# sair-lab/AirSLAM

Hardware: AMD Instinct MI355X
Metric: stereo detect+match pairs/sec (2x PLNet @512x512 internal: points + lines, junctions on the left + LightGlue match) (higher is better)
Workload: dtype fp16

## Files before the change

### airslam_amd/_lib.py

```python
from __future__ import annotations

import ctypes as C
import os

_HERE = os.path.dirname(os.path.abspath(__file__))
LIB_PATH = os.path.join(_HERE, "libairfe.so")


class Tuning(C.Structure):
    _fields_ = [(n, C.c_int) for n in (
        "fuse_lg_block", "gemm_small_max_m", "gemm8_min_m", "gemmr_min_m", "gemmr_wgs", "qkv_pair", "block_min_m", "lgb_tokens", "sg_kenc_gemm",
        "fold_qkv", "overlap_lines", "kf_graph", "kf_spec_rows", "fuse_dec", "assign_fused", "fold_out_proj", "desc_gather_stream", "copy_wgs")] + [("reserved", C.c_int * 5)]


class Cfg(C.Structure):
    _fields_ = [
        ("device", C.c_int), ("precision", C.c_int), ("max_batch", C.c_int), ("enc_chunk", C.c_int),
        ("max_keypoints", C.c_int), ("keypoint_threshold", C.c_float), ("remove_borders", C.c_int),
        ("nms_radius", C.c_int), ("line_threshold", C.c_float), ("line_length_threshold", C.c_float),
        ("matcher", C.c_int), ("image_width", C.c_int), ("image_height", C.c_int), ("sinkhorn_iters", C.c_int),
        ("superpoint_pack", C.c_char_p), ("plnet_s1_pack", C.c_char_p), ("lightglue_pack", C.c_char_p),
        ("superglue_pack", C.c_char_p), ("matcher_precision", C.c_int), ("line_precision", C.c_int), ("check_launches", C.c_int),
        ("tuning", C.POINTER(Tuning)),
    ]


class Stage0(C.Structure):
# ... 188 lines not shown
    "airfe_stereo_points": (C.c_int, [C.c_void_p, C.c_void_p, C.c_void_p, C.c_int, C.c_void_p, C.c_int, C.c_void_p, C.c_int, C.c_void_p, C.c_void_p,
                                      C.c_void_p, C.POINTER(C.c_int)]),
    "airfe_stereo_points_batch_dev": (C.c_int, [C.c_void_p] * 6 + [C.c_int, C.c_int, C.c_void_p, C.c_void_p, C.c_int] + [C.c_void_p] * 5),
    "airfe_track_pose_batch_dev": (C.c_int, [C.c_void_p, C.c_void_p, C.c_void_p, C.c_int, C.c_void_p, C.c_int, C.c_void_p, C.c_void_p, C.c_int, C.c_int,
                                             C.c_void_p, C.c_void_p, C.c_void_p, C.c_void_p, C.c_void_p]),
    "airfe_frame_optimize": (C.c_int, [C.c_void_p, C.c_void_p, C.c_void_p, C.c_int] + [C.c_void_p] * 7 + [C.POINTER(C.c_int)]),
    "airfe_frame_optimize_batch_dev": (C.c_int, [C.c_void_p, C.c_void_p, C.c_void_p, C.c_void_p, C.c_int, C.c_int] + [C.c_void_p] * 9),
    "airfe_track_pose_opt_batch_dev": (C.c_int, [C.c_void_p, C.c_void_p, C.c_void_p, C.c_int, C.c_void_p, C.c_int, C.c_void_p, C.c_int, C.c_void_p,
                                                 C.c_void_p, C.c_int, C.c_int] + [C.c_void_p] * 9),
    "airfe_sync": (C.c_int, [C.c_void_p]),
    "airfe_superglue_status": (C.c_int, [C.c_void_p, C.c_void_p]),
    "airfe_profile_enable": (C.c_int, [C.c_void_p, C.c_int]),
    "airfe_profile_stages": (C.c_int, []),
    "airfe_profile_stage_name": (C.c_char_p, [C.c_int]),
    "airfe_profile_read": (C.c_int, [C.c_void_p, C.c_void_p, C.c_void_p, C.c_void_p, C.c_void_p]),
    "airfe_debug_detector_maps": (C.c_int, [C.c_void_p, C.c_int, C.c_void_p, C.c_void_p, C.c_void_p]),
    "airfe_debug_lightglue_scores": (C.c_int, [C.c_void_p, C.c_void_p, C.c_int, C.c_void_p, C.c_int, C.c_void_p]),
    "airfe_debug_superglue_scores": (C.c_int, [C.c_void_p, C.c_void_p, C.c_int, C.c_void_p, C.c_int, C.c_void_p]),
    "airfe_debug_lg_filter": (C.c_int, [C.c_void_p, C.c_void_p, C.c_int, C.c_int, C.c_void_p, C.c_void_p, C.c_int, C.POINTER(C.c_int)]),
    "airfe_debug_sg_decode": (C.c_int, [C.c_void_p, C.c_void_p, C.c_int, C.c_int, C.c_void_p, C.c_void_p, C.c_void_p, C.c_void_p]),
    "airfe_debug_sg_sinkhorn": (C.c_int, [C.c_void_p, C.c_void_p, C.c_void_p, C.c_int, C.c_int, C.c_float, C.c_int, C.c_int, C.c_void_p, C.POINTER(C.c_int)]),
    "airfe_debug_lg_prepare": (C.c_int, [C.c_void_p, C.POINTER(DebugLgPrepareArgs)]),
    "airfe_debug_lg_assign": (C.c_int, [C.c_void_p, C.POINTER(DebugLgAssignArgs)]),
    "airfe_debug_plnet_stage0": (C.c_int, [C.c_void_p] + [C.c_void_p] * 10),
    "airfe_debug_plnet_s1": (C.c_int, [C.c_void_p, C.POINTER(Stage0), C.c_void_p, C.c_void_p, C.c_int, C.POINTER(C.c_int)]),
    "airfe_debug_plnet_s1_last": (C.c_int, [C.c_void_p, C.c_void_p, C.c_void_p, C.c_int, C.POINTER(C.c_int)]),
    "airfe_debug_preprocess": (C.c_int, [C.c_void_p, C.c_void_p, C.c_int, C.c_int, C.c_int, C.c_void_p]),
    "airfe_debug_conv3x3": (C.c_int, [C.c_void_p, C.c_void_p, C.c_int, C.c_int, C.c_int, C.c_int, C.c_void_p, C.c_void_p,
                                      C.c_int, C.c_int, C.c_void_p]),
    "airfe_debug_conv": (C.c_int, [C.c_void_p, C.POINTER(DebugConvArgs)]),
# ... 38 lines not shown
```

### airslam_amd/api.py

```python
from __future__ import annotations

import ctypes as C
import os
import tempfile
from typing import Dict, Optional

import numpy as np

from . import _lib, weights as W

FEAT = 259


def _pack_arg(x, tmpfiles) -> Optional[bytes]:
    if x is None:
        return None
    if isinstance(x, (str, bytes, os.PathLike)):
        return os.fsencode(x)
    f = tempfile.NamedTemporaryFile(suffix=".airfe", delete=False)
    f.close()
    W.save_pack(f.name, x)
    tmpfiles.append(f.name)
    return f.name.encode()

# ... 387 lines not shown
                                   thr=float(thr), form=int(form), **{k: v.ctypes.data for k, v in out.items()})
        if pad is not None:
            pad = f32(pad)
            a.pad = pad.ctypes.data
        self._chk(self._l.airfe_debug_lg_assign(self._h, C.byref(a)), "airfe_debug_lg_assign")
        return out

    def detector_maps(self, b: int = 1):
        heat = np.empty((b, 512, 512), np.float32)
        nms = np.empty((b, 512, 512), np.float32)
        desc = np.empty((b, 64, 64, 256), np.float32)
        self._chk(self._l.airfe_debug_detector_maps(self._h, b, heat.ctypes.data, nms.ctypes.data, desc.ctypes.data),
                  "airfe_debug_detector_maps")
        return heat, nms, desc

    def debug_preprocess(self, gray):
        gray = np.ascontiguousarray(gray, np.uint8)
        out = np.empty((512, 512), np.float32)
        self._chk(self._l.airfe_debug_preprocess(self._h, gray.ctypes.data, gray.shape[0], gray.shape[1], gray.strides[0],
                                                 out.ctypes.data), "airfe_debug_preprocess")
        return out

    def debug_conv3x3(self, x, w, b, pool=False):
        x = np.ascontiguousarray(x, np.float32); w = np.ascontiguousarray(w, np.float32); b = np.ascontiguousarray(b, np.float32)
        bb, cin, hh, ww = x.shape
        cout = w.shape[0]
        ho, wo = (hh // 2, ww // 2) if pool else (hh, ww)
        y = np.empty((bb, cout, ho, wo), np.float32)
        self._chk(self._l.airfe_debug_conv3x3(self._h, x.ctypes.data, bb, cin, hh, ww, w.ctypes.data, b.ctypes.data, cout,
                                              int(pool), y.ctypes.data), "airfe_debug_conv3x3")
# ... 667 lines not shown
```

### airslam_amd/csrc/airfe.hip

```cpp
#include "airfe_host.h"

namespace airfe_host {
thread_local std::string g_err;

int fail(airfe_ctx* c, const std::string& m) {
  if (c) c->err = m;
  g_err = m;
  return 1;
}

int fail_noexcept(airfe_ctx* c, const char* what, const char* detail) noexcept {
  try {
    std::string m = std::string("airfe: C++ exception at the C boundary (") + what + "): " + (detail ? detail : "unknown");
    if (c) c->err = m;
    g_err = m;
  } catch (...) {
  }
  return 1;
}

int launch_status(airfe_ctx* c) {
  std::string m;
  if (c->launch_err.empty()) {
    const hipError_t e = hipGetLastError();
// ... 158 lines not shown
    if (t->qkv_pair >= 0) c->qkv_pair = t->qkv_pair != 0;
    if (t->block_min_m >= 0) c->block_min = t->block_min_m;
    if (t->lgb_tokens >= 0) {
      if (t->lgb_tokens != 32 && t->lgb_tokens != 64 && t->lgb_tokens != 112 && t->lgb_tokens != 128) { return fail(nullptr, "airfe_create: tuning.lgb_tokens must be 32, 64, 112 or 128"); }
      c->lgb_tokens = t->lgb_tokens;
    }
    if (t->sg_kenc_gemm >= 0) c->sg_kenc_gemm = t->sg_kenc_gemm != 0;
    if (t->fold_qkv >= 0) c->fold_qkv = t->fold_qkv != 0;
    if (t->overlap_lines >= 0) c->overlap_lines = t->overlap_lines != 0;
    if (t->kf_graph >= 0) c->kf_graph_on = t->kf_graph != 0;
    if (t->kf_spec_rows >= 0) c->kf_spec_lines = c->kf_spec_juncs = std::max(t->kf_spec_rows, 1);
    if (t->fuse_dec >= 0) c->fuse_dec = t->fuse_dec != 0;
    if (t->assign_fused >= 0) c->assign_fused = t->assign_fused != 0 ? 1 : 0;
    if (t->fold_out_proj >= 0) c->fold_out = t->fold_out_proj != 0;
    if (t->desc_gather_stream >= 0) c->desc_gather_stream = t->desc_gather_stream != 0;
    if (t->copy_wgs > 0) c->copy_wgs = t->copy_wgs;
  }
  if (hipStreamCreateWithFlags(&c->stream, hipStreamNonBlocking) != hipSuccess ||
      hipStreamCreateWithFlags(&c->stream2, hipStreamNonBlocking) != hipSuccess ||
      hipEventCreateWithFlags(&c->ev_fork, hipEventDisableTiming) != hipSuccess ||
      hipEventCreateWithFlags(&c->ev_join, hipEventDisableTiming) != hipSuccess ||
      hipEventCreateWithFlags(&c->ev_feat, hipEventDisableTiming) != hipSuccess)
    return fail(nullptr, "airfe_create: stream creation failed");
  c->Dmax = (c->prec != 2 && cfg->superpoint_pack && cfg->lightglue_pack) ? 2 * c->Bmax : c->Bmax;
  c->chunk = std::min(std::max(cfg->enc_chunk, 1), c->Dmax);
  c->Lmax = c->Dmax;
  int rc = 0;
  if (cfg->superpoint_pack) rc = load_superpoint(c, cfg->superpoint_pack);
  if (!rc && cfg->lightglue_pack) rc = load_lightglue(c, cfg->lightglue_pack);
  if (!rc && cfg->superglue_pack) rc = load_superglue(c, cfg->superglue_pack);
// ... 585 lines not shown
  }
  if (nlines) *nlines = nl;
  if (njunc) *njunc = nj;
  return 0;
} AIRFE_CATCH(c)

static int plnet_lines_batch(airfe_ctx* c, int B, int h, int w, double* d_lines, int capL, int* d_nlines, float* d_junc, int capJ,
                             int* d_njunc, int nj, int* d_found, hipStream_t st, int phase = 3) {
  if (!c->has_s0 || !c->has_s1) return fail(c, "the batched PLNet path needs the line branch (line.* in the detector pack) and cfg.plnet_s1_pack");
  if (c->prec == 2) return fail(c, "plnet_lines_batch is the 2-byte batch path (fp32 mode goes image by image: plnet_batch_f32)");
  if (B > c->Lmax) return fail(c, "batch exceeds the line-path arena");
  if (capL < 1 || !d_lines || !d_nlines) return fail(c, "detect_plnet_batch: no line output");
  if (nj < 0 || nj > B || (nj > 0 && (!d_junc || !d_njunc || capJ < 1))) return fail(c, "detect_plnet_batch: bad junction arguments");
  if ((phase & 1) && line_branch_dev(c, st, 0, B, false)) return 1;
  bool partial = false;
  if ((phase & 2) && nj > 0 && !c->desc_dense_valid) {
    dense_desc_head(c, nj, st);
    c->desc_dense_valid = true;
    partial = nj != c->last_B;
  }
  int* lfound = d_found ? d_found : c->d_nlines + c->Lmax;
  int* jfound = d_found ? d_found + B : c->d_njunc + c->Lmax;
  const int rc = line_tail_dev(c, 0, B, nullptr, h, w, d_lines, capL, d_nlines, lfound, d_junc, capJ, d_njunc, jfound, nj, st, phase);
  if (partial) c->desc_dense_valid = false;
  return rc;
}

static int plnet_batch_f32(airfe_ctx* c, const uint8_t* d_gray, int B, int h, int w, int stride, size_t img_stride, float* d_feat, int cap, int* d_n,
                           double* d_lines, int capL, int* d_nlines, float* d_junc, int capJ, int* d_njunc, int nj, int* lfound, int* jfound, hipStream_t st) {
  if (!c->has_s0 || !c->has_s1) return fail(c, "the batched PLNet path needs the line branch (line.* in the detector pack) and cfg.plnet_s1_pack");
  if (capL < 1 || !d_lines || !d_nlines) return fail(c, "detect_plnet_batch: no line output");
  if (nj < 0 || nj > B || (nj > 0 && (!d_junc || !d_njunc || capJ < 1))) return fail(c, "detect_plnet_batch: bad junction arguments");
  for (int b = 0; b < B; ++b) {
    const bool jn = b < nj;
    const int rc = detect_dev(c, d_gray + (size_t)b * img_stride, 1, h, w, stride, img_stride, d_feat + (size_t)b * cap * AIRFE_FEAT_DIM, cap, d_n + b, st);
    if (rc || line_branch_dev(c, st, 0, 1, false)) return 1;
    if (line_tail_dev(c, 0, 1, nullptr, h, w, d_lines + (size_t)b * capL * 4, capL, d_nlines + b, lfound ? lfound + b : c->d_nlines + c->Lmax,
                      jn ? d_junc + (size_t)b * capJ * AIRFE_FEAT_DIM : nullptr, capJ, jn ? d_njunc + b : nullptr, jn ? (jfound ? jfound + b : c->d_njunc + c->Lmax) : nullptr,
// ... 570 lines not shown
```

### airslam_amd/csrc/airfe_debug.hip

```cpp
#include "airfe_host.h"

struct DbgTmp {
  airfe_ctx h;
  DbgTmp() {}
  explicit DbgTmp(int prec) { h.prec = h.pack_prec = prec; }
  ~DbgTmp() { for (void* p : h.allocs) (void)hipFree(p); }
};

static std::vector<uint16_t> dbg_conv_x(const float* x, int B, int cin, int H, int W, int prec) {
  std::vector<uint16_t> xin((size_t)B * (H + 2) * (W + 2) * cin, 0);
  for (int bb = 0; bb < B; ++bb)
    for (int ci = 0; ci < cin; ++ci)
      for (int yy = 0; yy < H; ++yy)
        for (int xx = 0; xx < W; ++xx)
          xin[(((size_t)bb * (H + 2) + yy + 1) * (W + 2) + xx + 1) * cin + ci] = cvt2(x[(((size_t)bb * cin + ci) * H + yy) * W + xx], prec);
  return xin;
}
static std::vector<uint16_t> dbg_conv_slabs(const float* w, int cin, int cout, int prec) {
  const int nci = cin / 64;
  return pack_slabs(cout / 64, 9 * nci, prec, [&](int feat, int s, int k) {
    const int tap = s / nci, cc = s % nci, ci = cc * 64 + k;
    return w[((size_t)feat * cin + ci) * 9 + tap];
  });
}
// ... 618 lines not shown
  HIPCHK(c, hipMemcpy2D(a->rowlse, nb, c->rowlse, npb, nb, B, hipMemcpyDeviceToHost));
  HIPCHK(c, hipMemcpy2D(a->collse, nb, c->collse, npb, nb, B, hipMemcpyDeviceToHost));
  HIPCHK(c, hipMemcpy2D(a->rowval, nb, c->rowval, npb, nb, B, hipMemcpyDeviceToHost));
  HIPCHK(c, hipMemcpy2D(a->rowarg, nb, c->rowarg, npb, nb, B, hipMemcpyDeviceToHost));
  HIPCHK(c, hipMemcpy2D(a->colarg, nb, c->colarg, npb, nb, B, hipMemcpyDeviceToHost));
  HIPCHK(c, hipMemcpy(a->idx, didx, (size_t)B * cap * 8, hipMemcpyDeviceToHost));
  HIPCHK(c, hipMemcpy(a->score, dscore, (size_t)B * cap * 4, hipMemcpyDeviceToHost));
  HIPCHK(c, hipMemcpy(a->nmatch, dnm, (size_t)B * 4, hipMemcpyDeviceToHost));
  HIPCHK(c, hipMemsetAsync(c->mdb, 0, M * 256 * 2, st));
  HIPCHK(c, hipMemsetAsync(c->x32, 0, M * 256 * 4, st));
  HIPCHK(c, hipMemsetAsync(c->zbuf, 0, M * 4, st));
  HIPCHK(c, hipStreamSynchronize(st));
  return 0;
} AIRFE_CATCH(c)

}
```

### airslam_amd/csrc/airfe_detect.hip

```cpp
#include "airfe_host.h"

namespace airfe_host {

int ensure_tables(airfe_ctx* c, int h, int w) {
  if (c->tab_w == w && c->tab_h == h) return 0;
  const auto xt = resize_table(AIRFE_INTERNAL_SIZE, w), yt = resize_table(AIRFE_INTERNAL_SIZE, h);
  if (c->tab_w != -1) HIPCHK(c, hipDeviceSynchronize());
  HIPCHK(c, hipMemcpyAsync(c->xtab, xt.data(), xt.size() * 4, hipMemcpyHostToDevice, c->stream));
  HIPCHK(c, hipMemcpyAsync(c->ytab, yt.data(), yt.size() * 4, hipMemcpyHostToDevice, c->stream));
  HIPCHK(c, hipStreamSynchronize(c->stream));
  c->tab_w = w;
  c->tab_h = h;
  return 0;
}

int run_conv(airfe_ctx* c, const ConvW& w, const uint16_t* x, uint16_t* y, int B, int H, int W, int pool, int out_pad,
             hipStream_t st) {
  ConvArgs a;
  a.X = x; a.Wp = w.w; a.bias = w.b; a.Y = y;
  a.B = B; a.H = H; a.W = W; a.CIN = w.cin; a.COUT = w.cout;
  a.pool = pool; a.out_pad = out_pad; a.relu = 1;
  const double px = (double)B * H * W;
  const double ob = px / (pool ? 4 : 1) * w.cout * 2;
  {
// ... 40 lines not shown
}

int dense_desc_head(airfe_ctx* c, int B, hipStream_t st) {
  const int R = AIRFE_INTERNAL_SIZE, cells = B * (R / 8) * (R / 8);
  GemmArgs g;
  g.X1 = c->aDa; g.ld1 = 256; g.K1 = 256; g.Wp = c->cDb.w; g.bias = c->cDb.b;
  g.M = cells; g.N = 256; g.cb_total = c->cDb.cbt; g.epi = EPI_STORE_F32; g.out = c->desc; g.ldo = 256;
  g.small_max = c->gemm_small_max; g.g8_min = c->gemm8_min; g.gr_min = c->gemmr_min; g.gr_wgs = c->gemmr_wgs;
  {
    ProfScope ps(c, ST_HEAD_GEMM, st, 2.0 * cells * 256 * 256, (double)cells * (512 + 1024));
    if (c->desc_gather_stream && cells >= c->gemmr_min && gemmr_gather_applicable(256, g)) launch_gemmr_gather(c->prec, g, st);
    else launch_gemm(c->prec, 256, false, g, st);
  }
  c->desc_normalised = false;
  return c->cfg.check_launches ? launch_status(c) : 0;
}

int detect_dev2(airfe_ctx* c, const uint8_t* d_gray, const uint8_t* d_gray1, int Bs, int h, int w, int stride, size_t img_stride,
                float* d_feat, float* d_feat1, int cap, int* d_n, int* d_n1, hipStream_t st) {
  if (!c->has_sp) return fail(c, "detector weights were not loaded (cfg.superpoint_pack)");
  const int B = d_gray1 ? 2 * Bs : Bs;
  if (Bs < 1 || Bs > c->Bmax || B > c->Dmax) return fail(c, "batch exceeds cfg.max_batch");
  if (h < 1 || w < 1) return fail(c, "empty image");
  if (cap < c->cfg.max_keypoints) return fail(c, "feature capacity < max_keypoints");
  if (ensure_tables(c, h, w)) return 1;
  const int R = AIRFE_INTERNAL_SIZE;
  bool sparse_desc = false;
  if (c->prec == 2) {
    if (d_gray1) return fail(c, "detect_dev2: the fp32 path takes one source");
    if (encode_f32(c, d_gray, B, h, w, stride, img_stride, st)) return 1;
// ... 138 lines not shown
    launch_s0_decode(c->l_head, 160, 128, d + SG_LP, c->l_jloc, nullptr, c->l_joff, d + SG_THIN, d + SG_AUX, chw ? c->s0_loi : nullptr, c->l_ta8, nb,
                     SG_STRIDE, st);
  else
    launch_s0_decode(c->l_dec, 32, 0, d + SG_LP, c->l_jloc, nullptr, c->l_joff, d + SG_THIN, d + SG_AUX, nullptr, c->l_ta8, nb, SG_STRIDE, st);
  const int ccap = F * F;
  hipStream_t s3 = st;
  launch_candidates_nms3(c->l_jloc, nb, F, F, 1e-30f, c->l_cand, c->l_cand_cnt, ccap, s3);
  launch_select_list(c->l_cand, c->l_cand_cnt, ccap, nb, F, 300, 320, c->l_sel, c->l_nsel, s3);
  launch_s0_juncs(c->l_sel, c->l_nsel, c->l_joff, d + SG_JUNCS, 300, 320, nb, SG_STRIDE, s3);
  c->wf_counted = launch_s0_j2l(d + SG_LP, d + SG_JUNCS, 300, NP, 10.0f, d + SG_KEEP, d + SG_MIN, d + SG_MAX, c->wf_counts, nb, SG_STRIDE, chw ? 1 : 0, s3);
  }
  return launch_status(c);
}

int line_tail_dev(airfe_ctx* c, int i0, int nb, const float* loi_chw, int h, int w, double* d_lines, int capL, int* d_nlines, int* d_lfound,
                  float* d_junc, int capJ, int* d_njunc, int* d_jfound, int nj, hipStream_t st, int phase) {
  if (!c->has_s1) return fail(c, "PLNet stage-1 weights were not loaded (cfg.plnet_s1_pack)");
  if (nb < 1 || nb > c->Lmax || nj < 0 || nj > nb) return fail(c, "line path: image range outside the arena");
  const int R = AIRFE_INTERNAL_SIZE, NP = KEEP_CAP;
  float* d = c->s0_stage;
  const float ws = (float)w / (float)R, hs = (float)h / (float)R;
  if (phase & 1) {
  hipStream_t s4 = st;
  if (nj > 0) launch_zero16(c->jmap, (size_t)nj * R * R, s4);
  {
  ProfScope ps(c, ST_PL_STAGE1, st, 0, (double)nb * 49152 * 12);
  launch_wireframe(d + SG_KEEP, d + SG_MIN, d + SG_MAX, NP, 300, c->wf_table, c->wf_keep, c->wf_pairs, c->wf_rep, KEEP_CAP, LINE_CAP,
                   c->wf_counts, c->wf_counted, d + SG_JUNCS, d + SG_LP, c->s1_la, c->wf_prop, nb, SG_STRIDE, s4);
  c->wf_counted = false;
  if (loi_chw) {
    launch_plnet_s1(d + SG_JUNCS, d + SG_LP, c->wf_keep, c->wf_pairs, c->wf_rep, c->wf_counts, loi_chw, 0, nullptr, nullptr, d + SG_THIN, d + SG_AUX,
// ... 15 lines not shown
    } else {
      launch_s1_junc_proj(d + SG_JUNCS, c->l_head, (size_t)128 * 128 * 160, 160, nullptr, 300, c->s1_w[0], c->s1_jfeat, nb, SG_STRIDE, st);
    }
    if (c->cfg.line_precision == 3)
      launch_plnet_s1h(c->wf_pairs, c->wf_counts, c->s1_jfeat, c->l_ta8, c->s1_wsplit, c->s1_w, c->s1_la, c->wf_prop, c->s1_sc, LINE_CAP, nb, st);
    else
      launch_plnet_s1(d + SG_JUNCS, d + SG_LP, c->wf_keep, c->wf_pairs, c->wf_rep, c->wf_counts, nullptr, 0, c->s1_jfeat, c->l_ta8, d + SG_THIN,
                      d + SG_AUX, c->s1_w, c->s1_la, c->s1_sc, KEEP_CAP, LINE_CAP, nb, SG_STRIDE, st);
  }
  }
  ProfScope ps(c, ST_PL_FILTER, st, 0, (double)nb * R * R);
  launch_line_filter(c->s1_la, c->s1_sc, c->wf_counts, c->cfg.remove_borders, c->cfg.line_threshold, c->cfg.line_length_threshold, ws, hs, R,
                     c->jmap, nj, d_lines, capL, d_nlines, d_lfound, LINE_CAP, nb, st);
  }
  if ((phase & 2) && nj > 0) {
    ProfScope ps(c, ST_PL_FILTER, st, 0, (double)nj * R * R * 2);
    const bool from_mask = c->cfg.nms_radius > 0 && !c->nms_map_valid;
    if (from_mask && c->cfg.nms_radius != 4) return fail(c, "line path: the NMS'd score maps of this batch were not kept");
    const float* hsel = (c->cfg.nms_radius > 0 && !from_mask ? c->heat_nms : c->heat) + (size_t)i0 * R * R;
    const unsigned long long* mask = from_mask ? reinterpret_cast<const unsigned long long*>(c->nms_mask) + (size_t)i0 * (R / 8) * (R / 8) : nullptr;
    launch_junction_scan(c->jmap, hsel, R, c->cfg.remove_borders, d_junc, capJ, d_njunc, d_jfound, c->d_njunc + 2 * c->Lmax, nj, st, mask);
    if (!c->desc_dense_valid) return fail(c, "line path: the dense descriptor map of this batch was not made");
    launch_sample_desc(c->desc + (size_t)i0 * (R / 8) * (R / 8) * 256, nj, R / 8, R / 8, d_junc, d_njunc, capJ, ws, hs,
                       c->desc_normalised ? 0 : 1, st);
  }
  return launch_status(c);
}

}
```

### airslam_amd/csrc/airfe_host.h

```cpp
#pragma once
#include "../../include/airfe.h"
#include "../../include/airfe_debug.h"

#include <hip/hip_runtime.h>

#include <algorithm>
#include <cmath>
#include <cstdio>
#include <cstdlib>
#include <cstring>
#include <functional>
#include <map>
#include <string>
#include <vector>

#include "kernels.h"
#include "common.h"

using namespace airfe;


namespace airfe_host {

extern thread_local std::string g_err;
// ... 99 lines not shown
  bool outlier_rejection = false;
  bool nms_map_valid = true;
  int Lmax = 1;
  bool desc_normalised = false;
  int gemm_small_max = 4096, gemm8_min = 16000, gemmr_min = 8192, gemmr_wgs = 256;
  int block_min = 0;
  bool qkv_pair = true;
  int fuse_lg_block = -1;
  int sg_kenc_gemm = -1;
  bool desc_dense_valid = true;
  int last_B = 0;
  int* desc_idx = nullptr;
  int n_cu = 0;
  bool fold_qkv = true;
  bool desc_gather_stream = true;
  bool fold_out = true;

  float *c1a_w = nullptr, *c1a_b = nullptr;
  ConvW c1b, c2a, c2b, c3a, c3b, c4a, c4b, cPa, cDa;
  LinW cPb, cDb;
  float* img32 = nullptr;
  uint16_t *a1b = nullptr, *a2a = nullptr, *a2b = nullptr, *a3a = nullptr, *a3b = nullptr, *a4a = nullptr,
           *a4b = nullptr, *aPa = nullptr, *aDa = nullptr;
  float *logits = nullptr, *heat = nullptr, *heat_nms = nullptr, *nms_tmp = nullptr, *desc = nullptr;
  unsigned char* nms_mask = nullptr;
  int *xtab = nullptr, *ytab = nullptr;
  float* lut = nullptr;
  unsigned long long* cand = nullptr;
  int* cand_cnt = nullptr;
  int tab_w = -1, tab_h = -1;
// ... 180 lines not shown
  uint32_t u = (uint32_t)v << 16;
  float f;
  memcpy(&f, &u, 4);
  return f;
}
bool make_linear(airfe_ctx* c, const float* W, const float* bias, int K, int N, LinW& out, float scale = 1.f,
                 const std::function<int(int)>* src_row = nullptr, const std::function<int(int)>* src_col = nullptr);
int ensure_tables(airfe_ctx* c, int h, int w);
int run_conv(airfe_ctx* c, const ConvW& w, const uint16_t* x, uint16_t* y, int B, int H, int W, int pool, int out_pad, hipStream_t st);
int dense_desc_head(airfe_ctx* c, int B, hipStream_t st);
int detect_dev2(airfe_ctx* c, const uint8_t* d_gray, const uint8_t* d_gray1, int Bs, int h, int w, int stride, size_t img_stride,
                float* d_feat, float* d_feat1, int cap, int* d_n, int* d_n1, hipStream_t st);
int detect_dev(airfe_ctx* c, const uint8_t* d_gray, int B, int h, int w, int stride, size_t img_stride, float* d_feat, int cap, int* d_n, hipStream_t st);
int line_branch_dev(airfe_ctx* c, hipStream_t st, int i0, int nb, bool chw);
int line_tail_dev(airfe_ctx* c, int i0, int nb, const float* loi_chw, int h, int w, double* d_lines, int capL, int* d_nlines, int* d_lfound,
                  float* d_junc, int capJ, int* d_njunc, int* d_jfound, int nj, hipStream_t st, int phase = 3);
void trace(airfe_ctx* c, hipStream_t st, const char* what, size_t li, const char* blk, const void* p, size_t words, unsigned unit_words);
int trace_finish(airfe_ctx* c, hipStream_t st);
int run_linear(airfe_ctx* c, const LinW& w, const uint16_t* x1, int ld1, int K1, const uint16_t* x2, int ld2, int M, int epi, int act, void* out,
                int ldo, hipStream_t st, bool trans = false, void* out2 = nullptr, float* x32 = nullptr, const float* rc = nullptr, const float* rs = nullptr);
void reset_slack_rows(airfe_ctx* c, int M, hipStream_t st);
struct LgSecondPair { const float *f0, *f1; const int *n0, *n1; };
int lightglue_dev(airfe_ctx* c, const float* f0, const int* n0, const float* f1, const int* n1, int B, int cap, int ld, int kp_off, int normalize,
                  int32_t* d_idx, float* d_score, int mcap, int* d_nmatch, float* scores_out, hipStream_t st, const LgSecondPair* x2 = nullptr);
int superglue_dev(airfe_ctx* c, const float* f0, const int* n0, const float* f1, const int* n1, int B, int cap, int normalize, hipStream_t st);

}

#define AIRFE_CATCH(c)                                                                                                   \
  catch (const std::exception& e_) { return airfe_host::fail_noexcept((c), __func__, e_.what()); }                       \
  catch (...) { return airfe_host::fail_noexcept((c), __func__, nullptr); }
// ... 29 lines not shown
```

### airslam_amd/csrc/gemmr_body.h

```cpp
#pragma once
#include "common.h"
#include "kernels.h"
#include "desc_sample.h"

namespace airfe {

constexpr int GR_MT = 2;
constexpr int GR_TT = 16 * GR_MT;
constexpr int GR_XBYTES = GR_TT * 512;
constexpr int GR_RBYTES = 2 * GR_TT * 128;

template <int N>
__device__ __forceinline__ void gr_wait_vm() { asm volatile("s_waitcnt vmcnt(%0)" ::"n"(N) : "memory"); }

__device__ __forceinline__ void gr_glds16(const void* gsrc, unsigned lds_off) {
  unsigned keep;
  asm volatile("s_mov_b32 %0, m0\n\ts_mov_b32 m0, %2\n\ts_nop 0\n\tglobal_load_lds_dwordx4 %1, off\n\ts_mov_b32 m0, %0"
               : "=&s"(keep)
               : "v"(gsrc), "s"(lds_off)
               : "memory");
}

constexpr int GR_SAMPLE_SLOTS = 7;
constexpr int GR_STAGE_LD = 260;
constexpr int GR_STAGE_BYTES = GR_TT * GR_STAGE_LD * 4;
struct GrKeypoint { float x, y; int row, second; };

template <class P, bool TRANS, bool ROT, bool GATHER = false, bool SAMPLE = false>
__device__ __forceinline__ void gemmr_body(const GemmArgs& a, char* smem, int group, int first, int per_group, int ntiles, const DescSample* dsp = nullptr) {
  static_assert(!GATHER || (!TRANS && !ROT), "the gather form is the plain K = 256 linear with fp32 rows out");
  static_assert(!SAMPLE || GATHER, "sampling finishes the gather form's rows");
  constexpr int GR_SLOT = GR_XBYTES + (ROT ? GR_RBYTES : 0);
  constexpr int GR_SLOTS = ROT ? 6 : SAMPLE ? GR_SAMPLE_SLOTS : 8;
  constexpr int PER = ROT ? 3 : 2;
  const int tid = threadIdx.x, lane = tid & 63, l15 = lane & 15, g = lane >> 4;
  const int wave = __builtin_amdgcn_readfirstlane(tid >> 6);
  const int n = first < ntiles ? (ntiles - first + per_group - 1) / per_group : 0;
  if (n == 0) return;

  const int cb = group * 4 + (wave >> 1), tp = wave & 1;
  typename P::vec8 wreg[2][8];
  {
    const int sw = (l15 >> 1) & 7;
    const char* wb = reinterpret_cast<const char*>(a.Wp) + (size_t)cb * 4 * SLAB_BYTES + 2 * tp * 2048 + l15 * 128;
#pragma unroll
    for (int u = 0; u < 2; ++u)
#pragma unroll
      for (int ks = 0; ks < 8; ++ks)
        wreg[u][ks] = __builtin_bit_cast(typename P::vec8, *reinterpret_cast<const uint4*>(
            wb + u * 2048 + (ks >> 1) * SLAB_BYTES + ((((ks & 1) * 4 + g) ^ sw) << 4)));
  }
  f32x4 binit[2];
  float bt[2];
#pragma unroll
  for (int u = 0; u < 2; ++u) {
    binit[u] = *reinterpret_cast<const f32x4*>(a.bias + cb * 64 + tp * 32 + g * 8 + u * 4);
    bt[u] = a.bias[cb * 64 + slab_row_to_feature((2 * tp + u) * 16 + l15)];
  }
  [[maybe_unused]] float* stage = reinterpret_cast<float*>(smem + GR_SLOTS * GR_SLOT);
  [[maybe_unused]] int* idx_lds = reinterpret_cast<int*>(smem + GR_SLOTS * GR_SLOT + (SAMPLE ? GR_STAGE_BYTES : 0));
  [[maybe_unused]] GrKeypoint* kp_lds = reinterpret_cast<GrKeypoint*>(idx_lds + n * GR_TT);
  if constexpr (GATHER) {
    for (int e = tid; e < n * GR_TT; e += 512) {
      const int r = (first + (e >> 5) * per_group) * GR_TT + (e & 31);
      idx_lds[e] = a.rowidx ? a.rowidx[r] : r;
    }
  }
  if constexpr (SAMPLE) {
    const DescSample& ds = *dsp;
    for (int e = tid; e < n * 8; e += 512) {
      const int s = (first + (e >> 3) * per_group) * 8 + (e & 7);
      const int b = s / ds.cap, k = s - b * ds.cap;
      GrKeypoint kp{0.f, 0.f, -1, 0};
      if (b < ds.B) {
        const bool second = ds.feat1 && b >= ds.Bs;
        const int bl = second ? b - ds.Bs : b;
        if (k < (second ? ds.n1 : ds.n)[bl]) {
          const float* f = (second ? ds.feat1 : ds.feat) + ((size_t)bl * ds.cap + k) * 259;
          kp.row = bl * ds.cap + k;
          kp.second = second ? 1 : 0;
          kp.x = f[1];
          kp.y = f[2];
        }
// ... 129 lines not shown
```

### airslam_amd/csrc/kernels.h

```cpp
#pragma once
#include <hip/hip_runtime.h>
#include <stdint.h>

namespace airfe {

enum Epi {
  EPI_STORE = 0,
  EPI_STORE_F32 = 1,
  EPI_RESID = 2,
  EPI_HEADS = 3,
  EPI_HEADS_T = 4,
  EPI_SOFTMAX_D2S = 5
};
enum Act { ACT_NONE = 0, ACT_RELU = 1 };

struct GemmArgs {
  const uint16_t* X1 = nullptr;
  const uint16_t* X2 = nullptr;
  int ld1 = 0, ld2 = 0, K1 = 0;
  const uint16_t* Wp = nullptr;
  const float* bias = nullptr;
  int M = 0;
  int N = 0;
  int cb_total = 0;
// ... 80 lines not shown
  float* feat1 = nullptr; int* n_out1 = nullptr; int Bs = 0;
  int* desc_idx = nullptr; int HC = 0, WC = 0;
};
void launch_select_list(const unsigned long long* cand, const int* cand_cnt, int cand_cap, int B, int W, int topk, int cap,
                        float* feat, int* n_out, hipStream_t st, const SelectExtra* ex = nullptr);
void launch_sample_desc(const float* desc, int B, int HC, int WC, float* feat, const int* n, int cap,
                        float w_scale, float h_scale, int normalise, hipStream_t st, int compact = 0, int* flag = nullptr,
                        float* feat1 = nullptr, const int* n1 = nullptr, int Bs = 0);
struct DescSample {
  float* feat = nullptr; float* feat1 = nullptr;
  const int* n = nullptr; const int* n1 = nullptr;
  int Bs = 0, B = 0, cap = 0, HC = 0, WC = 0;
  float w_scale = 1.f, h_scale = 1.f;
  int* flag = nullptr;
  float sx = 0.f, bx = 0.f, sy = 0.f, by = 0.f;
};
bool gemmr_gather_sample_applicable(const GemmArgs& a);
void launch_gemmr_gather_sample(int prec, const GemmArgs& a, const DescSample& ds, hipStream_t st);

struct LgPrepArgs {
  const float* f0; const float* f1;
  const int* n0; const int* n1;
  int ld, kp_off;
  int normalize;
  float cx, cy, linv;
  const float* wr;
  int B, cap, Np;
  float* x32; uint16_t* xb;
  float* rot_cos; float* rot_sin;
  int* lens;
  const float *f0x = nullptr, *f1x = nullptr; const int *n0x = nullptr, *n1x = nullptr;
  int slack_rows = 0;
};
// ... 314 lines not shown
```

### airslam_amd/csrc/kernels_gemmr_sample.hip

```cpp
#include "gemmr_body.h"

namespace airfe {

template <class P>
__global__ __launch_bounds__(512, 1) void gemmr_gather_kernel_sample(GemmArgs a, int ntiles, DescSample ds) {
  extern __shared__ __attribute__((aligned(16))) char smem[];
  gemmr_body<P, false, false, true, true>(a, smem, 0, blockIdx.x, gridDim.x, ntiles, &ds);
}


constexpr int GR_SAMPLE_MAX_TILES = 60;
bool gemmr_gather_sample_applicable(const GemmArgs& a) {
  const int wgs = std::max(a.gr_wgs, 1);
  return gemmr_gather_applicable(256, a) && a.rowidx && (a.M / GR_TT + wgs - 1) / wgs <= GR_SAMPLE_MAX_TILES;
}

void launch_gemmr_gather_sample(int prec, const GemmArgs& a, const DescSample& ds0, hipStream_t st) {
  DescSample ds = ds0;
  desc_grid_coeffs(ds.HC, ds.WC, ds.sx, ds.bx, ds.sy, ds.by);
  const int ntiles = a.M / GR_TT;
  const int nwg = std::max(std::min(a.gr_wgs, ntiles), 1);
  const int nmax = (ntiles + nwg - 1) / nwg;
  const int lds = GR_SAMPLE_SLOTS * GR_XBYTES + GR_STAGE_BYTES + nmax * (GR_TT * 4 + 8 * (int)sizeof(GrKeypoint));
  if (prec == 1) {
    static PerDeviceOnce once;
    if (auto once_token = once.first()) (void)hipFuncSetAttribute(reinterpret_cast<const void*>(gemmr_gather_kernel_sample<PF16>), hipFuncAttributeMaxDynamicSharedMemorySize, 160 * 1024);
    hipLaunchKernelGGL(gemmr_gather_kernel_sample<PF16>, dim3((unsigned)nwg), dim3(512), lds, st, a, ntiles, ds);
  } else {
    static PerDeviceOnce once;
    if (auto once_token = once.first()) (void)hipFuncSetAttribute(reinterpret_cast<const void*>(gemmr_gather_kernel_sample<PBF16>), hipFuncAttributeMaxDynamicSharedMemorySize, 160 * 1024);
    hipLaunchKernelGGL(gemmr_gather_kernel_sample<PBF16>, dim3((unsigned)nwg), dim3(512), lds, st, a, ntiles, ds);
  }
}

}
```

### include/airfe.h

```cpp
#ifndef AIRFE_H_
#define AIRFE_H_

#include <stddef.h>
#include <stdint.h>

#ifdef __cplusplus
extern "C" {
#endif

#define AIRFE_FEAT_DIM 259
#define AIRFE_INTERNAL_SIZE 512

typedef struct airfe_ctx airfe_ctx;

typedef struct airfe_tuning {
  int fuse_lg_block;
  int gemm_small_max_m;
  int gemm8_min_m;
  int gemmr_min_m;
  int gemmr_wgs;
  int qkv_pair;
  int block_min_m;
  int lgb_tokens;
  int sg_kenc_gemm;
  int fold_qkv;
  int overlap_lines;
  int kf_graph;
  int kf_spec_rows;
  int fuse_dec;
  int assign_fused;
  int fold_out_proj;
  int desc_gather_stream;
  int copy_wgs;
  int reserved[5];
} airfe_tuning;

typedef struct airfe_cfg {
  int device;
  int precision;
  int max_batch;
  int enc_chunk;
  int max_keypoints;
  float keypoint_threshold;
  int remove_borders;
  int nms_radius;
  float line_threshold;
  float line_length_threshold;
  int matcher;
  int image_width;
// ... 226 lines not shown
```

### include/airfe_debug.h

```cpp
#ifndef AIRFE_DEBUG_H_
#define AIRFE_DEBUG_H_
#include "airfe.h"
#ifdef __cplusplus
extern "C" {
#endif

int airfe_debug_detector_maps(airfe_ctx* ctx, int B, float* heat_raw, float* heat_nms, float* desc);
int airfe_debug_lightglue_scores(airfe_ctx* ctx, const float* f0, int n0, const float* f1, int n1, float* scores);
int airfe_debug_lg_filter(airfe_ctx* ctx, const float* scores, int n0, int n1, int32_t* idx, float* score, int cap, int* nmatch);
int airfe_debug_sg_decode(airfe_ctx* ctx, const float* Z, int n0, int n1, int32_t* idx0, int32_t* idx1, double* ms0, double* ms1);
int airfe_debug_sg_sinkhorn(airfe_ctx* ctx, const float* sim, const int* lens , int B, int ld ,
                            float alpha, int iters, int form , float* Z , int* form_ran);
int airfe_debug_superglue_scores(airfe_ctx* ctx, const float* f0, int n0, const float* f1, int n1, float* scores);
int airfe_debug_plnet_stage0(airfe_ctx* ctx, float* juncs_pred, float* lines_pred, float* iskeep, float* idx_min, float* idx_max,
                             float* loi, float* thin, float* aux, float* jloc, float* joff);
int airfe_debug_plnet_j2l(airfe_ctx* ctx, int fast, float* iskeep, float* idx_min, float* idx_max);
int airfe_debug_plnet_s1(airfe_ctx* ctx, const airfe_plnet_stage0* stage0, float* lines_adjusted, float* scores_line,
                         int cap, int* m2);
int airfe_debug_plnet_s1_last(airfe_ctx* ctx, float* lines_adjusted, float* scores_line, int cap, int* m2);
int airfe_debug_preprocess(airfe_ctx* ctx, const uint8_t* gray, int h, int w, int stride, float* out);
int airfe_debug_conv3x3(airfe_ctx* ctx, const float* x, int B, int cin, int H, int W, const float* w, const float* b,
                        int cout, int pool, float* y);
int airfe_debug_gemm(airfe_ctx* ctx, const float* x, int M, int K, const float* w, const float* b, int N, int relu, float* y);
typedef struct airfe_debug_conv_args {
// ... 97 lines not shown
  float b;
  const int* lens;
  int cap;
  float thr;
  int form;
  const float* pad;
  float* z;
  float *sim, *scores;
  float *rowlse, *collse, *rowval;
  int32_t *rowarg, *colarg;
  int32_t* idx;
  float* score;
  int32_t* nmatch;
} airfe_debug_lg_assign_args;
int airfe_debug_lg_assign(airfe_ctx* ctx, airfe_debug_lg_assign_args* a);
int airfe_debug_fail_next_launch(airfe_ctx* ctx, int stage);
int airfe_debug_trace(airfe_ctx* ctx, int on);
int airfe_debug_trace_stop(airfe_ctx* ctx, int slot);
int airfe_debug_trace_buffer(airfe_ctx* ctx, int slot, void* host, size_t bytes);
int airfe_debug_trace_slots(airfe_ctx* ctx);
int airfe_debug_trace_slot(airfe_ctx* ctx, int i, char* name, int name_cap, unsigned* off, unsigned* units, unsigned* unit_words);
int airfe_debug_trace_read(airfe_ctx* ctx, void* stream, unsigned long long* digests, unsigned long long* table);

#ifdef __cplusplus
}
#endif
#endif
```

Baseline: 7778.

## Compute junction descriptors sparsely via fused gather-GEMM instead of dense head

Junction descriptors on the left image are now produced by a fused gather GEMM that runs the descriptor head only on the four bilinear tap rows of each detected junction. Before, the full dense descriptor head ran over every 64x64 cell and was then sampled. A count-aware tile list skips tiles past each image's junction count, and a host heuristic picks the workgroup count to balance load. The dense path stays as a fallback when the dense map is already valid or the sparse path does not apply. Taps can repeat across junctions, and the per-junction work depends on how many junctions are found.

```diff
diff --git a/airslam_amd/_lib.py b/airslam_amd/_lib.py
--- a/airslam_amd/_lib.py
+++ b/airslam_amd/_lib.py
@@ -11,6 +11,7 @@
     _fields_ = [(n, C.c_int) for n in (
         "fuse_lg_block", "gemm_small_max_m", "gemm8_min_m", "gemmr_min_m", "gemmr_wgs", "qkv_pair", "block_min_m", "lgb_tokens", "sg_kenc_gemm",
         "fold_qkv", "overlap_lines", "kf_graph", "kf_spec_rows", "fuse_dec", "assign_fused", "fold_out_proj", "desc_gather_stream", "copy_wgs")] + [("reserved", C.c_int * 5)]
+    junc_desc_sparse = property(lambda self: self.reserved[0], lambda self, v: self.reserved.__setitem__(0, int(v)))
 
 
 class Cfg(C.Structure):
@@ -229,6 +230,7 @@
     "airfe_profile_stages": (C.c_int, []),
     "airfe_profile_stage_name": (C.c_char_p, [C.c_int]),
     "airfe_profile_read": (C.c_int, [C.c_void_p, C.c_void_p, C.c_void_p, C.c_void_p, C.c_void_p]),
+    "airfe_debug_junction_desc": (C.c_int, [C.c_void_p, C.c_void_p, C.c_int, C.c_void_p, C.c_int, C.c_void_p, C.c_int, C.c_int, C.c_int, C.c_int, C.POINTER(C.c_int)]),
     "airfe_debug_detector_maps": (C.c_int, [C.c_void_p, C.c_int, C.c_void_p, C.c_void_p, C.c_void_p]),
     "airfe_debug_lightglue_scores": (C.c_int, [C.c_void_p, C.c_void_p, C.c_int, C.c_void_p, C.c_int, C.c_void_p]),
     "airfe_debug_superglue_scores": (C.c_int, [C.c_void_p, C.c_void_p, C.c_int, C.c_void_p, C.c_int, C.c_void_p]),
diff --git a/airslam_amd/api.py b/airslam_amd/api.py
--- a/airslam_amd/api.py
+++ b/airslam_amd/api.py
@@ -425,6 +425,16 @@
                   "airfe_debug_detector_maps")
         return heat, nms, desc
 
+    def debug_junction_desc(self, act, junc, n, w=512, h=512, form=1):
+        act = np.ascontiguousarray(act, np.uint16)
+        out = np.array(junc, order="C", copy=True)
+        n = np.ascontiguousarray(n, np.int32)
+        assert act.ndim == 3 and act.shape[1:] == (4096, 256) and out.ndim == 3 and out.shape[2] == 259 and out.itemsize == 4 and n.shape == (out.shape[0],)
+        ran = C.c_int(0)
+        self._chk(self._l.airfe_debug_junction_desc(self._h, act.ctypes.data, act.shape[0], out.ctypes.data, out.shape[1], n.ctypes.data, out.shape[0], int(w), int(h),
+                                                    int(form), C.byref(ran)), "airfe_debug_junction_desc")
+        return out, bool(ran.value)
+
     def debug_preprocess(self, gray):
         gray = np.ascontiguousarray(gray, np.uint8)
         out = np.empty((512, 512), np.float32)
diff --git a/airslam_amd/csrc/airfe.hip b/airslam_amd/csrc/airfe.hip
--- a/airslam_amd/csrc/airfe.hip
+++ b/airslam_amd/csrc/airfe.hip
@@ -196,6 +196,7 @@
     if (t->assign_fused >= 0) c->assign_fused = t->assign_fused != 0 ? 1 : 0;
     if (t->fold_out_proj >= 0) c->fold_out = t->fold_out_proj != 0;
     if (t->desc_gather_stream >= 0) c->desc_gather_stream = t->desc_gather_stream != 0;
+    if (t->junc_desc_sparse >= 0) c->junc_desc_sparse = t->junc_desc_sparse != 0;
     if (t->copy_wgs > 0) c->copy_wgs = t->copy_wgs;
   }
   if (hipStreamCreateWithFlags(&c->stream, hipStreamNonBlocking) != hipSuccess ||
@@ -811,14 +812,15 @@
   if (nj < 0 || nj > B || (nj > 0 && (!d_junc || !d_njunc || capJ < 1))) return fail(c, "detect_plnet_batch: bad junction arguments");
   if ((phase & 1) && line_branch_dev(c, st, 0, B, false)) return 1;
   bool partial = false;
-  if ((phase & 2) && nj > 0 && !c->desc_dense_valid) {
+  const int junc_wgs = (phase & 2) && nj > 0 ? junc_desc_sparse_wgs(c, nj, capJ) : 0;
+  if ((phase & 2) && nj > 0 && !c->desc_dense_valid && junc_wgs == 0) {
     dense_desc_head(c, nj, st);
     c->desc_dense_valid = true;
     partial = nj != c->last_B;
   }
   int* lfound = d_found ? d_found : c->d_nlines + c->Lmax;
   int* jfound = d_found ? d_found + B : c->d_njunc + c->Lmax;
-  const int rc = line_tail_dev(c, 0, B, nullptr, h, w, d_lines, capL, d_nlines, lfound, d_junc, capJ, d_njunc, jfound, nj, st, phase);
+  const int rc = line_tail_dev(c, 0, B, nullptr, h, w, d_lines, capL, d_nlines, lfound, d_junc, capJ, d_njunc, jfound, nj, st, phase, junc_wgs);
   if (partial) c->desc_dense_valid = false;
   return rc;
 }
diff --git a/airslam_amd/csrc/airfe_debug.hip b/airslam_amd/csrc/airfe_debug.hip
--- a/airslam_amd/csrc/airfe_debug.hip
+++ b/airslam_amd/csrc/airfe_debug.hip
@@ -656,4 +656,38 @@
   return 0;
 } AIRFE_CATCH(c)
 
-}
+int airfe_debug_junction_desc(airfe_ctx* c, const uint16_t* act, int B, float* junc, int capJ, const int* n, int nj, int w, int h, int form, int* ran_sparse) try {
+  AIRFE_ENTER(c);
+  if (!c->has_sp || c->prec == 2) return fail(c, "debug_junction_desc: needs the detector in a 2-byte storage type");
+  if (!act || !junc || !n || B < 1 || B > c->Dmax || nj < 1 || nj > B || capJ < 1 || w < 1 || h < 1) return fail(c, "debug_junction_desc: bad arguments");
+  for (int b = 0; b < nj; ++b)
+    if (n[b] < 0 || n[b] > capJ) return fail(c, "debug_junction_desc: count outside [0, capJ]");
+  const int R = AIRFE_INTERNAL_SIZE;
+  const size_t cells = (size_t)(R / 8) * (R / 8), words = (size_t)nj * capJ * AIRFE_FEAT_DIM;
+  hipStream_t st = c->stream;
+  DbgTmp t;
+  float* d_junc = dalloc<float>(&t.h, words, false);
+  int* d_n = dalloc<int>(&t.h, (size_t)nj, false);
+  if (!d_junc || !d_n) return fail(c, "debug_junction_desc: allocation failed");
+  HIPCHK(c, hipMemcpyAsync(c->aDa, act, (size_t)B * cells * 256 * 2, hipMemcpyHostToDevice, st));
+  HIPCHK(c, hipMemcpyAsync(d_junc, junc, words * 4, hipMemcpyHostToDevice, st));
+  HIPCHK(c, hipMemcpyAsync(d_n, n, (size_t)nj * 4, hipMemcpyHostToDevice, st));
+  c->desc_dense_valid = false;
+  c->last_B = B;
+  const float ws = (float)w / (float)R, hs = (float)h / (float)R;
+  const int wgs = form ? junc_desc_sparse_wgs(c, nj, capJ) : 0;
+  if (wgs > 0) {
+    junc_desc_sparse(c, 0, nj, d_junc, capJ, d_n, ws, hs, wgs, st);
+  } else {
+    if (dense_desc_head(c, nj, st)) return 1;
+    launch_sample_desc(c->desc, nj, R / 8, R / 8, d_junc, d_n, capJ, ws, hs, 1, st);
+    c->desc_dense_valid = nj == B;
+  }
+  HIPCHK(c, hipStreamSynchronize(st));
+  if (launch_status(c)) return 1;
+  HIPCHK(c, hipMemcpy(junc, d_junc, words * 4, hipMemcpyDeviceToHost));
+  if (ran_sparse) *ran_sparse = wgs > 0 ? 1 : 0;
+  return 0;
+} AIRFE_CATCH(c)
+
+}
diff --git a/airslam_amd/csrc/airfe_detect.hip b/airslam_amd/csrc/airfe_detect.hip
--- a/airslam_amd/csrc/airfe_detect.hip
+++ b/airslam_amd/csrc/airfe_detect.hip
@@ -78,6 +78,29 @@
   }
   c->desc_normalised = false;
   return c->cfg.check_launches ? launch_status(c) : 0;
+}
+
+int junc_desc_sparse_wgs(airfe_ctx* c, int nj, int capJ) {
+  if (!c->junc_desc_sparse || !c->desc_gather_stream || c->desc_dense_valid || c->prec == 2 || nj < 1) return 0;
+  if (c->junc_wgs_key[0] != nj || c->junc_wgs_key[1] != capJ || c->junc_wgs_key[2] != c->gemmr_wgs) {
+    c->junc_wgs = junc_desc_wgs(nj, capJ, c->gemmr_wgs);
+    c->junc_wgs_key[0] = nj; c->junc_wgs_key[1] = capJ; c->junc_wgs_key[2] = c->gemmr_wgs;
+  }
+  if (c->junc_wgs < 1) return 0;
+  GemmArgs g;
+  g.ld1 = 256; g.K1 = 256; g.M = nj * capJ * 4; g.N = 256; g.cb_total = c->cDb.cbt; g.epi = EPI_STORE_F32; g.ldo = 256; g.gr_wgs = c->junc_wgs;
+  return gemmr_gather_applicable(256, g) ? c->junc_wgs : 0;
+}
+
+void junc_desc_sparse(airfe_ctx* c, int i0, int nj, float* d_junc, int capJ, const int* d_njunc, float ws, float hs, int wgs, hipStream_t st) {
+  const int R = AIRFE_INTERNAL_SIZE;
+  GemmArgs g;
+  g.X1 = c->aDa; g.ld1 = 256; g.K1 = 256; g.Wp = c->cDb.w; g.bias = c->cDb.b;
+  g.M = nj * capJ * 4; g.N = 256; g.cb_total = c->cDb.cbt; g.epi = EPI_STORE_F32; g.ldo = 256; g.gr_wgs = wgs;
+  DescSample ds;
+  ds.feat = d_junc; ds.n = d_njunc; ds.Bs = nj; ds.B = nj; ds.cap = capJ; ds.HC = R / 8; ds.WC = R / 8; ds.w_scale = ws; ds.h_scale = hs;
+  ds.src_row0 = i0 * (R / 8) * (R / 8);
+  launch_gemmr_gather_junc(c->prec, g, ds, st);
 }
 
 int detect_dev2(airfe_ctx* c, const uint8_t* d_gray, const uint8_t* d_gray1, int Bs, int h, int w, int stride, size_t img_stride,
@@ -246,7 +269,7 @@
 }
 
 int line_tail_dev(airfe_ctx* c, int i0, int nb, const float* loi_chw, int h, int w, double* d_lines, int capL, int* d_nlines, int* d_lfound,
-                  float* d_junc, int capJ, int* d_njunc, int* d_jfound, int nj, hipStream_t st, int phase) {
+                  float* d_junc, int capJ, int* d_njunc, int* d_jfound, int nj, hipStream_t st, int phase, int junc_wgs) {
   if (!c->has_s1) return fail(c, "PLNet stage-1 weights were not loaded (cfg.plnet_s1_pack)");
   if (nb < 1 || nb > c->Lmax || nj < 0 || nj > nb) return fail(c, "line path: image range outside the arena");
   const int R = AIRFE_INTERNAL_SIZE, NP = KEEP_CAP;
@@ -292,15 +315,19 @@
                      c->jmap, nj, d_lines, capL, d_nlines, d_lfound, LINE_CAP, nb, st);
   }
   if ((phase & 2) && nj > 0) {
-    ProfScope ps(c, ST_PL_FILTER, st, 0, (double)nj * R * R * 2);
+    ProfScope ps(c, ST_PL_FILTER, st, 0, (double)nj * R * R * 2 + (junc_wgs > 0 ? (double)nj * (capJ / 4) * (4 * 512 + 1036) : 0.0));
     const bool from_mask = c->cfg.nms_radius > 0 && !c->nms_map_valid;
     if (from_mask && c->cfg.nms_radius != 4) return fail(c, "line path: the NMS'd score maps of this batch were not kept");
     const float* hsel = (c->cfg.nms_radius > 0 && !from_mask ? c->heat_nms : c->heat) + (size_t)i0 * R * R;
     const unsigned long long* mask = from_mask ? reinterpret_cast<const unsigned long long*>(c->nms_mask) + (size_t)i0 * (R / 8) * (R / 8) : nullptr;
     launch_junction_scan(c->jmap, hsel, R, c->cfg.remove_borders, d_junc, capJ, d_njunc, d_jfound, c->d_njunc + 2 * c->Lmax, nj, st, mask);
-    if (!c->desc_dense_valid) return fail(c, "line path: the dense descriptor map of this batch was not made");
-    launch_sample_desc(c->desc + (size_t)i0 * (R / 8) * (R / 8) * 256, nj, R / 8, R / 8, d_junc, d_njunc, capJ, ws, hs,
-                       c->desc_normalised ? 0 : 1, st);
+    if (junc_wgs > 0) {
+      junc_desc_sparse(c, i0, nj, d_junc, capJ, d_njunc, ws, hs, junc_wgs, st);
+    } else {
+      if (!c->desc_dense_valid) return fail(c, "line path: the dense descriptor map of this batch was not made");
+      launch_sample_desc(c->desc + (size_t)i0 * (R / 8) * (R / 8) * 256, nj, R / 8, R / 8, d_junc, d_njunc, capJ, ws, hs,
+                         c->desc_normalised ? 0 : 1, st);
+    }
   }
   return launch_status(c);
 }
diff --git a/airslam_amd/csrc/airfe_host.h b/airslam_amd/csrc/airfe_host.h
--- a/airslam_amd/csrc/airfe_host.h
+++ b/airslam_amd/csrc/airfe_host.h
@@ -137,6 +137,8 @@
   int n_cu = 0;
   bool fold_qkv = true;
   bool desc_gather_stream = true;
+  bool junc_desc_sparse = true;
+  int junc_wgs_key[3] = {0, 0, 0}, junc_wgs = 0;
   bool fold_out = true;
 
   float *c1a_w = nullptr, *c1a_b = nullptr;
@@ -347,7 +349,9 @@
 int detect_dev(airfe_ctx* c, const uint8_t* d_gray, int B, int h, int w, int stride, size_t img_stride, float* d_feat, int cap, int* d_n, hipStream_t st);
 int line_branch_dev(airfe_ctx* c, hipStream_t st, int i0, int nb, bool chw);
 int line_tail_dev(airfe_ctx* c, int i0, int nb, const float* loi_chw, int h, int w, double* d_lines, int capL, int* d_nlines, int* d_lfound,
-                  float* d_junc, int capJ, int* d_njunc, int* d_jfound, int nj, hipStream_t st, int phase = 3);
+                  float* d_junc, int capJ, int* d_njunc, int* d_jfound, int nj, hipStream_t st, int phase = 3, int junc_wgs = 0);
+int junc_desc_sparse_wgs(airfe_ctx* c, int nj, int capJ);
+void junc_desc_sparse(airfe_ctx* c, int i0, int nj, float* d_junc, int capJ, const int* d_njunc, float ws, float hs, int wgs, hipStream_t st);
 void trace(airfe_ctx* c, hipStream_t st, const char* what, size_t li, const char* blk, const void* p, size_t words, unsigned unit_words);
 int trace_finish(airfe_ctx* c, hipStream_t st);
 int run_linear(airfe_ctx* c, const LinW& w, const uint16_t* x1, int ld1, int K1, const uint16_t* x2, int ld2, int M, int epi, int act, void* out,
diff --git a/airslam_amd/csrc/gemmr_body.h b/airslam_amd/csrc/gemmr_body.h
--- a/airslam_amd/csrc/gemmr_body.h
+++ b/airslam_amd/csrc/gemmr_body.h
@@ -26,17 +26,18 @@
 constexpr int GR_STAGE_BYTES = GR_TT * GR_STAGE_LD * 4;
 struct GrKeypoint { float x, y; int row, second; };
 
-template <class P, bool TRANS, bool ROT, bool GATHER = false, bool SAMPLE = false>
+template <class P, bool TRANS, bool ROT, bool GATHER = false, bool SAMPLE = false, bool COUNTED = false>
 __device__ __forceinline__ void gemmr_body(const GemmArgs& a, char* smem, int group, int first, int per_group, int ntiles, const DescSample* dsp = nullptr) {
   static_assert(!GATHER || (!TRANS && !ROT), "the gather form is the plain K = 256 linear with fp32 rows out");
   static_assert(!SAMPLE || GATHER, "sampling finishes the gather form's rows");
+  static_assert(!COUNTED || SAMPLE, "the count-aware tile list belongs to the sampling form");
   constexpr int GR_SLOT = GR_XBYTES + (ROT ? GR_RBYTES : 0);
   constexpr int GR_SLOTS = ROT ? 6 : SAMPLE ? GR_SAMPLE_SLOTS : 8;
   constexpr int PER = ROT ? 3 : 2;
   const int tid = threadIdx.x, lane = tid & 63, l15 = lane & 15, g = lane >> 4;
   const int wave = __builtin_amdgcn_readfirstlane(tid >> 6);
-  const int n = first < ntiles ? (ntiles - first + per_group - 1) / per_group : 0;
-  if (n == 0) return;
+  const int ncap = first < ntiles ? (ntiles - first + per_group - 1) / per_group : 0;
+  if (ncap == 0) return;
 
   const int cb = group * 4 + (wave >> 1), tp = wave & 1;
   typename P::vec8 wreg[2][8];
@@ -59,14 +60,47 @@
   }
   [[maybe_unused]] float* stage = reinterpret_cast<float*>(smem + GR_SLOTS * GR_SLOT);
   [[maybe_unused]] int* idx_lds = reinterpret_cast<int*>(smem + GR_SLOTS * GR_SLOT + (SAMPLE ? GR_STAGE_BYTES : 0));
-  [[maybe_unused]] GrKeypoint* kp_lds = reinterpret_cast<GrKeypoint*>(idx_lds + n * GR_TT);
-  if constexpr (GATHER) {
+  [[maybe_unused]] GrKeypoint* kp_lds = reinterpret_cast<GrKeypoint*>(idx_lds + ncap * GR_TT);
+  int nact = ncap;
+  [[maybe_unused]] int* tl = reinterpret_cast<int*>(stage);
+  if constexpr (COUNTED) {
+    const DescSample& ds = *dsp;
+    if (wave == 0) {
+      const int t = first + lane * per_group, s = t * 8, b = s / ds.cap;
+      const bool act = lane < ncap && b < ds.B && s - b * ds.cap < ds.n[b];
+      const unsigned long long m = __ballot(act);
+      if (act) tl[__popcll(m & ((1ull << lane) - 1ull))] = t;
+      if (lane == 0) tl[64] = __popcll(m);
+    }
+    __syncthreads();
+    nact = __builtin_amdgcn_readfirstlane(tl[64]);
+    if (nact == 0) return;
+    for (int e = tid; e < nact * 8; e += 512) {
+      const int s = tl[e >> 3] * 8 + (e & 7);
+      const int b = s / ds.cap, k = s - b * ds.cap;
+      GrKeypoint kp{0.f, 0.f, -1, 0};
+      int4 rows = make_int4(0, 0, 0, 0);
+      if (b < ds.B && k < ds.n[b]) {
+        const float* f = ds.feat + (size_t)s * 259;
+        kp.row = s;
+        kp.x = f[1];
+        kp.y = f[2];
+        const DescTaps tp = desc_taps(kp.x, kp.y, ds.sx, ds.bx, ds.sy, ds.by, ds.HC, ds.WC);
+        const int base = ds.src_row0 + b * ds.HC * ds.WC;
+        rows = make_int4(base + tp.c[0], base + tp.c[1], base + tp.c[2], base + tp.c[3]);
+      }
+      kp_lds[e] = kp;
+      *reinterpret_cast<int4*>(idx_lds + e * 4) = rows;
+    }
+  }
+  const int n = nact;
+  if constexpr (GATHER && !COUNTED) {
     for (int e = tid; e < n * GR_TT; e += 512) {
       const int r = (first + (e >> 5) * per_group) * GR_TT + (e & 31);
       idx_lds[e] = a.rowidx ? a.rowidx[r] : r;
     }
   }
-  if constexpr (SAMPLE) {
+  if constexpr (SAMPLE && !COUNTED) {
     const DescSample& ds = *dsp;
     for (int e = tid; e < n * 8; e += 512) {
       const int s = (first + (e >> 3) * per_group) * 8 + (e & 7);
diff --git a/airslam_amd/csrc/kernels.h b/airslam_amd/csrc/kernels.h
--- a/airslam_amd/csrc/kernels.h
+++ b/airslam_amd/csrc/kernels.h
@@ -118,9 +118,12 @@
   float w_scale = 1.f, h_scale = 1.f;
   int* flag = nullptr;
   float sx = 0.f, bx = 0.f, sy = 0.f, by = 0.f;
+  int src_row0 = 0;
 };
 bool gemmr_gather_sample_applicable(const GemmArgs& a);
 void launch_gemmr_gather_sample(int prec, const GemmArgs& a, const DescSample& ds, hipStream_t st);
+int junc_desc_wgs(int B, int cap, int max_wgs);
+void launch_gemmr_gather_junc(int prec, const GemmArgs& a, const DescSample& ds, hipStream_t st);
 
 struct LgPrepArgs {
   const float* f0; const float* f1;
diff --git a/airslam_amd/csrc/kernels_gemmr_sample.hip b/airslam_amd/csrc/kernels_gemmr_sample.hip
--- a/airslam_amd/csrc/kernels_gemmr_sample.hip
+++ b/airslam_amd/csrc/kernels_gemmr_sample.hip
@@ -8,6 +8,11 @@
   gemmr_body<P, false, false, true, true>(a, smem, 0, blockIdx.x, gridDim.x, ntiles, &ds);
 }
 
+template <class P>
+__global__ __launch_bounds__(512, 1) void gemmr_gather_kernel_junc(GemmArgs a, int ntiles, DescSample ds) {
+  extern __shared__ __attribute__((aligned(16))) char smem[];
+  gemmr_body<P, false, false, true, true, true>(a, smem, 0, blockIdx.x, gridDim.x, ntiles, &ds);
+}
 
 constexpr int GR_SAMPLE_MAX_TILES = 60;
 bool gemmr_gather_sample_applicable(const GemmArgs& a) {
@@ -33,4 +38,45 @@
   }
 }
 
+int junc_desc_wgs(int B, int cap, int max_wgs) {
+  if (B < 1 || cap < 8 || cap % 8 || cap > 1024 || max_wgs < 1) return 0;
+  const int T = cap / 8, ntiles = B * T, fill = std::max(T / 4, 1);
+  const int hi = std::min(max_wgs, ntiles), lo = std::max((hi + 1) / 2, (ntiles + GR_SAMPLE_MAX_TILES - 1) / GR_SAMPLE_MAX_TILES);
+  int best = 0, best_load = 1 << 30;
+  std::vector<int> d;
+  for (int w = hi; w >= lo; --w) {
+    d.assign(w + 1, 0);
+    int base = 0;
+    for (int b = 0; b < B; ++b) {
+      const int start = (int)(((long long)b * T) % w), rem = fill % w;
+      base += fill / w;
+      ++d[start];
+      if (start + rem <= w) --d[start + rem];
+      else { ++d[0]; --d[start + rem - w]; }
+    }
+    int load = 0, run = 0;
+    for (int i = 0; i < w; ++i) { run += d[i]; load = std::max(load, run); }
+    if (load + base < best_load) { best_load = load + base; best = w; }
+  }
+  return best;
 }
+
+void launch_gemmr_gather_junc(int prec, const GemmArgs& a, const DescSample& ds0, hipStream_t st) {
+  DescSample ds = ds0;
+  desc_grid_coeffs(ds.HC, ds.WC, ds.sx, ds.bx, ds.sy, ds.by);
+  const int ntiles = a.M / GR_TT;
+  const int nwg = std::max(std::min(a.gr_wgs, ntiles), 1);
+  const int nmax = (ntiles + nwg - 1) / nwg;
+  const int lds = GR_SAMPLE_SLOTS * GR_XBYTES + GR_STAGE_BYTES + nmax * (GR_TT * 4 + 8 * (int)sizeof(GrKeypoint));
+  if (prec == 1) {
+    static PerDeviceOnce once;
+    if (auto once_token = once.first()) (void)hipFuncSetAttribute(reinterpret_cast<const void*>(gemmr_gather_kernel_junc<PF16>), hipFuncAttributeMaxDynamicSharedMemorySize, 160 * 1024);
+    hipLaunchKernelGGL(gemmr_gather_kernel_junc<PF16>, dim3((unsigned)nwg), dim3(512), lds, st, a, ntiles, ds);
+  } else {
+    static PerDeviceOnce once;
+    if (auto once_token = once.first()) (void)hipFuncSetAttribute(reinterpret_cast<const void*>(gemmr_gather_kernel_junc<PBF16>), hipFuncAttributeMaxDynamicSharedMemorySize, 160 * 1024);
+    hipLaunchKernelGGL(gemmr_gather_kernel_junc<PBF16>, dim3((unsigned)nwg), dim3(512), lds, st, a, ntiles, ds);
+  }
+}
+
+}
diff --git a/include/airfe.h b/include/airfe.h
--- a/include/airfe.h
+++ b/include/airfe.h
@@ -32,7 +32,8 @@
   int fold_out_proj;
   int desc_gather_stream;
   int copy_wgs;
-  int reserved[5];
+  int junc_desc_sparse;
+  int reserved[4];
 } airfe_tuning;
 
 typedef struct airfe_cfg {
diff --git a/include/airfe_debug.h b/include/airfe_debug.h
--- a/include/airfe_debug.h
+++ b/include/airfe_debug.h
@@ -135,6 +135,7 @@
   int32_t* nmatch;
 } airfe_debug_lg_assign_args;
 int airfe_debug_lg_assign(airfe_ctx* ctx, airfe_debug_lg_assign_args* a);
+int airfe_debug_junction_desc(airfe_ctx* ctx, const uint16_t* act, int B, float* junc, int capJ, const int* n, int nj, int w, int h, int form, int* ran_sparse);
 int airfe_debug_fail_next_launch(airfe_ctx* ctx, int stage);
 int airfe_debug_trace(airfe_ctx* ctx, int on);
 int airfe_debug_trace_stop(airfe_ctx* ctx, int slot);
```

After: 7834, median of 4. Within noise of the previous version (+0.7%).
